# jamesdolezal/biscuit

Measured on NVIDIA B200. Metric: MC-dropout tiles/sec (Xception-UQ, T=30, 299^2), higher is better.
Workload: dtype bf16

## Files before the change

biscuit_b200/csrc/model.cu:

```cuda
#include <cuda.h>

#include <cmath>
#include <cstdlib>
#include <map>
#include <memory>

#include "common.cuh"
#include "gemm_sm100.cuh"
#include "layers.cuh"
#include "head_sm100.cuh"
#include "dwpipe_sm100.cuh"
#include "sepconv2d_sm100.cuh"
#include "sepmid_sm100.cuh"
#include "conv1_sm100.cuh"
#include "stain_sm100.cuh"

int bq_stain_launch(bq_ctx* ctx, const uint8_t* tiles_dev, int64_t n, int32_t px, const float* lut_dev, float* stats_dev,
                    const float target_means[3], const float target_stds[3], uint8_t* out_dev);

using bq::bf16;
using bq::GemmParams;

namespace {

// ... 131 lines not shown
    for (int c = 0; c < cin; ++c)
      for (int o = 0; o < cout; ++o)
        h[(size_t)o * ktot + t * cin + c] = f32_to_bf16_rne(k->data[((size_t)t * cin + c) * cout + o]);
  w.cin = cin; w.cout = cout; w.ktot = ktot;
  if ((rc = upload(ctx, w.w, h.data(), h.size() * 2))) return rc;
  return load_bn(ctx, ti, name + "_bn", cout, w);
}

int load_dense(bq_ctx* ctx, const TensorIndex& ti, const std::string& name, int cin, int cout, PwWeights& w) {
  const bq_named_tensor *k, *b;
  int rc;
  if ((rc = need(ctx, ti, name + "/kernel", {cin, cout}, &k)) || (rc = need(ctx, ti, name + "/bias", {cout}, &b))) return rc;
  std::vector<uint16_t> h((size_t)cout * cin);
  for (int c = 0; c < cin; ++c)
    for (int o = 0; o < cout; ++o) h[(size_t)o * cin + c] = f32_to_bf16_rne(k->data[(size_t)c * cout + o]);
  w.cin = cin; w.cout = cout; w.ktot = cin;
  if ((rc = upload(ctx, w.w, h.data(), h.size() * 2))) return rc;
  return upload(ctx, w.shift, b->data, cout * 4);
}

enum OpKind { OP_STATS, OP_CONV1, OP_GEMM, OP_DW, OP_POOLADD, OP_SUBSAMPLE, OP_GAP, OP_SEP2D, OP_SEPMID };

struct Op {
  OpKind kind;
  int stage = 0;
  std::string tag;
  const bf16* in = nullptr;
  const bf16* in2 = nullptr;
  bf16* out = nullptr;
  int H = 0, W = 0, C = 0, Ho = 0, Wo = 0, Cout = 0;
  int relu_in = 0, pad_top = 0, pad_left = 0;
  const float* dw = nullptr;
  bq::sep2d::Sep2dParams s2;
  bq::sepmid::SepMidParams sm;
  bool padded_out = false;
  int in_pitch = 0, out_pitch = 0;
  GemmParams gp;
  int rows_per_tile = 0;
  int blk_k = 64;
  CUtensorMap ta, tb, tc, tr;
  CUtensorMap tb2;
};

struct Arena {
  DevBuf buf[5];
  bf16* p(int i) { return (bf16*)buf[i].p; }
};

}

struct bq_model {
  bq_ctx* ctx = nullptr;
  bq_model_config cfg{};
  bool weights_loaded = false;
  bool use_simt = false;
  bool use_graph = true;
  cudaGraphExec_t backbone_graph = nullptr;
  int64_t graph_kernels = 0;
  bool sep_mid = true;
  DevBuf midbuf[4];
  int max_batch = 0;
  int px = 299;

  DevBuf conv1_w, conv1_scale, conv1_shift;
  DevBuf conv1_wtc, conv1_sumw;
  DevBuf conv1_affine, conv1_m0;
  PwWeights conv2;
  std::map<std::string, std::unique_ptr<SepWeights>> sep;
  std::map<std::string, std::unique_ptr<PwWeights>> res;
  std::vector<std::unique_ptr<PwWeights>> hidden;
  DevBuf w3, b3;

  DevBuf tiles_dev;
  DevBuf tiles_dev2;
  DevBuf tiles_f32[2];
  bool input_f32 = false;
  int norm_kind = 0;
  float norm_means[3] = {0, 0, 0}, norm_stds[3] = {1, 1, 1};
  DevBuf tiles_norm, norm_lut, norm_stats;
  const uint8_t* tiles_src = nullptr;
  cudaStream_t copy_stream = nullptr;
  cudaEvent_t copied[2] = {}, consumed[2] = {};
  DevBuf mean, inv_std;
  Arena arena;
  DevBuf feat, feat_bf16;
  DevBuf h_act[2];
  DevBuf a2;
  DevBuf a0;
  int sites = 6;
  int n_sites = 2, slot[3] = {-1, 0, 1};
  int mask_w = 0;
  DevBuf out_mean, out_std;
// ... 162 lines not shown
    if ((rc = make_tmap(ctx, &op.ta, A.p(0), (uint64_t)s1 * s1 * B, 32, 32, 128, 32))) return rc;
    if ((rc = make_tmap(ctx, &op.tb, m->conv2.w.p, 64, 288, 288, 64, 32))) return rc;
    if ((rc = make_tmap_nhwc(ctx, &op.tc, A.p(1), (uint64_t)B, (uint64_t)s2, (uint64_t)s2, 64, 1, 32, 32, false, true))) return rc;
    op.tr = op.ta; op.tb2 = op.tb;
    op.Ho = s2; op.Wo = s2; op.Cout = 64;
    m->plan.push_back(op);
  }
  X = 1;
  int H = s2, C = 64;

  int dw_rc = BQ_OK;
  int n_dw = 0;
  auto add_dw = [&](const bf16* in, bf16* out, int h, int c, int relu_in, const SepWeights& sw, int stage, int in_pitch = 0) {
    Op op; op.kind = OP_DW; op.stage = stage; op.in = in; op.out = out; op.H = h; op.W = h; op.C = c;
    op.relu_in = relu_in; op.dw = (const float*)sw.dw.p;
    const int CC = (c % 64 != 0) ? 56 : 64;
    int r = make_tmap_nhwc(ctx, &op.ta, in, (uint64_t)B, (uint64_t)h, (uint64_t)h, (uint64_t)c, bq::dwp::kHalo, bq::dwp::kHalo, CC,
                           false, false, (uint64_t)in_pitch);
    if (r && !dw_rc) dw_rc = r;
    op.tag = "dw" + std::to_string(n_dw++);
    op.Ho = h; op.Wo = h; op.Cout = c;
    m->plan.push_back(op);
  };
  auto add_gemm = [&](const bf16* a, int rows, const PwWeights& w, bf16* out, int relu, const bf16* resid, int stage,
                      const char* tag, int h, int cout) -> int {
    Op op; op.stage = stage;
    int r = make_gemm(m, op, a, rows, w, out, relu, resid);
    if (r) return r;
    if (tag) op.tag = tag;
    op.Ho = h; op.Wo = h; op.Cout = cout;
    m->plan.push_back(op);
    return BQ_OK;
  };
  auto add_sep = [&](const bf16* in, bf16* dw_tmp, int h, int cin, int relu_in, const SepWeights& sw, bf16* out, int relu_out,
                     const bf16* resid, int stage, const char* tag, int in_pitch = 0) -> int {
    if (!in_pitch && !m->use_simt && !resid && cin % 64 == 0 && cin <= 256 && (sw.pw.cout == 128 || sw.pw.cout == 256)) {
      Op op; op.kind = OP_SEP2D; op.stage = stage;
      if (tag) op.tag = tag;
      op.in = in; op.out = out; op.H = h; op.W = h; op.C = cin; op.Ho = h; op.Wo = h; op.Cout = sw.pw.cout;
      op.s2.n_img = B; op.s2.H = h; op.s2.W = h; op.s2.K = cin; op.s2.N = sw.pw.cout;
      op.s2.relu_in = relu_in; op.s2.relu_out = relu_out;
      op.s2.dw = (const float*)sw.dw.p; op.s2.scale = (const float*)sw.pw.scale.p; op.s2.shift = (const float*)sw.pw.shift.p;
      int r;
      if ((r = make_tmap_nhwc(ctx, &op.ta, in, (uint64_t)B, (uint64_t)h, (uint64_t)h, (uint64_t)cin, bq::sep2d::kHH, bq::sep2d::kHW, 64, false))) return r;
      if ((r = make_tmap(ctx, &op.tb, sw.pw.w.p, (uint64_t)sw.pw.cout, (uint64_t)cin, (uint64_t)cin, (uint32_t)sw.pw.cout, 64))) return r;
      if ((r = make_tmap_nhwc(ctx, &op.tc, out, (uint64_t)B, (uint64_t)h, (uint64_t)h, (uint64_t)sw.pw.cout, 2, bq::sep2d::kPW, 32, false, true))) return r;
      m->plan.push_back(op);
      return BQ_OK;
    }
    add_dw(in, dw_tmp, h, cin, relu_in, sw, stage, in_pitch);
    return add_gemm(dw_tmp, h * h, sw.pw, out, relu_out, resid, stage, tag, h, sw.pw.cout);
  };
  auto res_block = [&](int b, int cout1, int cout2, int relu_first, int stage, const bf16* padded_in = nullptr,
                       bf16* padded_out = nullptr) -> int {
    int t[4]; others(X, t);
    const int Ho = (H + 1) / 2;
    const bf16* xin = padded_in ? padded_in : A.p(X);
    const int in_pitch = padded_in ? bq::sepmid::kPitch : 0;
    const SepWeights& s1w = *m->sep.at("block" + std::to_string(b) + "_sepconv1");
    const SepWeights& s2w = *m->sep.at("block" + std::to_string(b) + "_sepconv2");
    const PwWeights& rw = *m->res.at("block" + std::to_string(b) + "_res");
    { Op op; op.kind = OP_SUBSAMPLE; op.stage = stage; op.in = xin; op.in_pitch = in_pitch; op.out = A.p(t[0]); op.H = H; op.W = H; op.Ho = Ho; op.Wo = Ho; op.C = C; m->plan.push_back(op); }
    int r;
    if ((r = add_gemm(A.p(t[0]), Ho * Ho, rw, A.p(t[1]), 0, nullptr, stage, nullptr, Ho, cout2))) return r;
    if ((r = add_sep(xin, A.p(t[0]), H, C, relu_first, s1w, A.p(t[2]), 1, nullptr, stage, nullptr, in_pitch))) return r;
    if ((r = add_sep(A.p(t[2]), A.p(t[0]), H, cout1, 0, s2w, A.p(t[3]), 0, nullptr, stage, nullptr))) return r;
    { Op op; op.kind = OP_POOLADD; op.stage = stage; op.in = A.p(t[3]); op.in2 = A.p(t[1]); op.out = padded_out ? padded_out : A.p(X);
      op.out_pitch = padded_out ? bq::sepmid::kPitch : 0; op.padded_out = padded_out != nullptr;
      op.H = H; op.W = H; op.Ho = Ho; op.Wo = Ho; op.C = cout2; op.Cout = cout2; op.pad_top = same_pad_before(H); op.pad_left = same_pad_before(H);
      op.tag = "block" + std::to_string(b); m->plan.push_back(op); }
    H = Ho; C = cout2;
    return BQ_OK;
  };
  if ((rc = res_block(2, 128, 128, 0, 2)) || (rc = res_block(3, 256, 256, 1, 2))) return rc;
  const bool mid = m->sep_mid && (H + 1) / 2 == bq::sepmid::kMap;
  auto P = [&](int i) { return (bf16*)m->midbuf[i].p; };
  if (mid) {
    using namespace bq::sepmid;
    const uint64_t rows = (uint64_t)B * kImgRows + kSlackRows;
    for (auto& b : m->midbuf) {
      if ((rc = bq_alloc(ctx, b, rows * kC * sizeof(bf16)))) return rc;
      BQ_CUDA(ctx, cudaMemset(b.p, 0, rows * kC * sizeof(bf16)));
    }
  }
  if ((rc = res_block(4, 728, 728, 1, 2, nullptr, mid ? P(0) : nullptr))) return rc;
  int mid_out = -1;
  if (mid) {
    using namespace bq::sepmid;
    const uint64_t rows = (uint64_t)B * kImgRows + kSlackRows;
    auto add_mid = [&](int src, int dst, int res, const SepWeights& sw, int relu_in, int relu_out, const char* tag) -> int {
      Op op; op.kind = OP_SEPMID; op.stage = 3; op.padded_out = true;
      if (tag) op.tag = tag;
      op.in = P(src); op.out = P(dst); op.in2 = res >= 0 ? P(res) : nullptr;
      op.H = kMap; op.W = kMap; op.C = kC; op.Ho = kMap; op.Wo = kMap; op.Cout = kC; op.relu_in = relu_in;
      op.sm.n_rows = B * kImgRows; op.sm.relu_out = relu_out;
      op.sm.dw = (const float*)sw.dw.p; op.sm.scale = (const float*)sw.pw.scale.p; op.sm.shift = (const float*)sw.pw.shift.p;
      op.sm.residual = op.in2;
      int r;
// ... 91 lines not shown
      KScope ks(m, g.conv_mode ? BQ_K_GEMM_CONV2 : BQ_K_GEMM_PW, 2.0 * rows_out * g.N * g.K,
                act * ((double)g.M * kin + rows_out * g.N * (g.residual ? 2 : 1) + (double)g.N * g.K));
      return launch_gemm(m, g, op.ta, op.tb, op.tc, op.tr, op.blk_k, g.conv_mode ? nullptr : &op.tb2);
    }
    case OP_DW: {
      KScope ks(m, BQ_K_DW, 2.0 * 9 * nb * op.H * op.W * op.C, 2 * act * nb * op.H * op.W * op.C);
      const int CC = (op.C % 64 != 0) ? 56 : 64;
      const int tiles = (op.H + bq::dwp::kTile - 1) / bq::dwp::kTile;
      const int64_t items = (int64_t)nb * tiles * tiles * (op.C / CC);
      const int grid = (int)std::min<int64_t>(items, ctx->num_sms);
#define BQ_DWP_LAUNCH(RELU, CCV)                                                                              \
  bq::dwp::depthwise3x3_pipe_kernel<RELU, CCV><<<grid, bq::dwp::kThreads, bq::dwp::kSmem, ctx->stream>>>(    \
      op.ta, op.dw, op.out, nb, op.H, op.W, op.C, tiles)
      if (CC == 56) { if (op.relu_in) BQ_DWP_LAUNCH(true, 56); else BQ_DWP_LAUNCH(false, 56); }
      else          { if (op.relu_in) BQ_DWP_LAUNCH(true, 64); else BQ_DWP_LAUNCH(false, 64); }
#undef BQ_DWP_LAUNCH
      break;
    }
    case OP_POOLADD: {
      KScope ks(m, BQ_K_POOLADD, 0, act * nb * op.C * ((double)op.H * op.W + 2.0 * op.Ho * op.Wo));
      bq::maxpool_add_kernel<<<grid1d((int64_t)nb * op.Ho * op.Wo * (op.C / 8)), 256, 0, ctx->stream>>>(
          op.in, op.in2, op.out + out_off, nb, op.H, op.W, op.Ho, op.Wo, op.C, op.pad_top, op.pad_left, op.out_pitch);
      break;
    }
    case OP_SUBSAMPLE: {
      KScope ks(m, BQ_K_SUBSAMPLE, 0, 2 * act * nb * op.Ho * op.Wo * op.C);
      bq::subsample2_kernel<<<grid1d((int64_t)nb * op.Ho * op.Wo * (op.C / 8)), 256, 0, ctx->stream>>>(
          op.in, op.out, nb, op.H, op.W, op.Ho, op.Wo, op.C, op.in_pitch);
      break;
    }
    case OP_SEP2D: {
      bq::sep2d::Sep2dParams s2 = op.s2;
      s2.n_img = nb;
      const int items = nb * ((op.H + bq::sep2d::kPH - 1) / bq::sep2d::kPH) * ((op.W + bq::sep2d::kPW - 1) / bq::sep2d::kPW);
      const int grid = items < ctx->num_sms ? items : ctx->num_sms;
      const double px_n = (double)nb * op.H * op.W;
      KScope ks(m, BQ_K_SEP_FUSED, 2.0 * px_n * s2.K * (s2.N + 9.0), act * px_n * (s2.K + s2.N));
      const int smem2d = bq::sep2d::smem_bytes(s2.N);
      if (s2.relu_in)
        bq::sep2d::sepconv2d_fused_kernel<true><<<grid, bq::sep2d::kThreads, smem2d, ctx->stream>>>(op.ta, op.tb, op.tc, s2);
      else
        bq::sep2d::sepconv2d_fused_kernel<false><<<grid, bq::sep2d::kThreads, smem2d, ctx->stream>>>(op.ta, op.tb, op.tc, s2);
      break;
    }
    case OP_SEPMID: {
      bq::sepmid::SepMidParams sm = op.sm;
      sm.n_rows = nb * bq::sepmid::kImgRows;
      const int items = (sm.n_rows + bq::sepmid::kItemPx - 1) / bq::sepmid::kItemPx;
      const int clusters = items < ctx->num_sms / 2 ? items : ctx->num_sms / 2;
      const double px_n = (double)nb * op.H * op.W;
      KScope ks(m, BQ_K_SEP_MID, 2.0 * px_n * op.C * (op.C + 9.0), act * px_n * op.C * (sm.residual ? 3.0 : 2.0));
      if (op.relu_in)
        bq::sepmid::sepconv_mid_kernel<true><<<2 * clusters, bq::sepmid::kThreads, bq::sepmid::kSmem, ctx->stream>>>(op.ta, op.tb, op.tc, op.tr, sm);
      else
        bq::sepmid::sepconv_mid_kernel<false><<<2 * clusters, bq::sepmid::kThreads, bq::sepmid::kSmem, ctx->stream>>>(op.ta, op.tb, op.tc, op.tr, sm);
      break;
    }
    case OP_GAP: {
      KScope ks(m, BQ_K_GAP, 0, act * nb * op.H * op.W * op.C + 6.0 * nb * op.C);
      bq::gap_kernel<<<grid1d((int64_t)nb * op.C), 256, 0, ctx->stream>>>(op.in, (float*)m->feat.p,
                                                                           (bf16*)m->feat_bf16.p, nb, op.H * op.W, op.C);
      break;
    }
  }
  BQ_LAUNCH_CHECK(ctx);
  return BQ_OK;
}

int stage_tiles(bq_model* m, const uint8_t* tiles, int nb) {
  bq_ctx* ctx = m->ctx;
  const size_t bytes = (size_t)nb * m->px * m->px * 3;
  BQ_CUDA(ctx, cudaMemcpyAsync(m->tiles_dev.p, tiles, bytes, cudaMemcpyDefault, ctx->stream));
  m->tiles_src = (const uint8_t*)m->tiles_dev.p;
  return BQ_OK;
}
// ... 153 lines not shown
    out[i] = __bfloat162float(in[i]);
}

}

extern "C" {

int bq_model_create(bq_ctx* ctx, const bq_model_config* cfg, bq_model** out) {
  if (!ctx) return BQ_ERR_ARG;
  if (!cfg || !out) return bq_fail(ctx, BQ_ERR_ARG, "bq_model_create: null argument");
  if (cfg->tile_px != 299) return bq_fail(ctx, BQ_ERR_ARG, "tile_px must be 299 (hp.py:5), got %d", cfg->tile_px);
  if (cfg->hidden_layers != 2) return bq_fail(ctx, BQ_ERR_ARG, "hidden_layers must be 2 (hp.py:21), got %d", cfg->hidden_layers);
  if (cfg->hidden_width <= 0 || cfg->hidden_width % 64) return bq_fail(ctx, BQ_ERR_ARG, "hidden_width must be a positive multiple of 64");
  if (cfg->n_classes < 2 || cfg->n_classes > bq::kMaxClasses) return bq_fail(ctx, BQ_ERR_ARG, "n_classes must be in [2,8]");
  if (!(cfg->dropout >= 0.f && cfg->dropout < 1.f)) return bq_fail(ctx, BQ_ERR_ARG, "dropout must be in [0,1)");
  if (cfg->max_batch < 1 || cfg->max_batch > 512) return bq_fail(ctx, BQ_ERR_ARG, "max_batch must be in [1,512]");
  BQ_CUDA(ctx, cudaSetDevice(ctx->device));
  bq_model* m = new bq_model();
  m->ctx = ctx;
  m->cfg = *cfg;
  m->max_batch = cfg->max_batch;
  m->px = cfg->tile_px;
  m->sites = cfg->dropout_sites ? cfg->dropout_sites : 6;
  if (m->sites & ~7) { delete m; return bq_fail(ctx, BQ_ERR_ARG, "dropout_sites must be a bitmask of sites 0..2"); }
  m->n_sites = 0;
  for (int i = 0; i < 3; ++i) m->slot[i] = (m->sites >> i) & 1 ? m->n_sites++ : -1;
  m->mask_w = (m->sites & 1) ? kFeatures : cfg->hidden_width;
  const char* g = getenv("BQ_GEMM");
  m->use_simt = g && strcmp(g, "simt") == 0;
  const char* gr = getenv("BQ_GRAPH");
  m->use_graph = !(gr && strcmp(gr, "off") == 0);
  const char* smid = getenv("BQ_SEPMID");
  m->sep_mid = !(smid && strcmp(smid, "off") == 0) && !m->use_simt;
  using namespace bq::sm100;
  cudaFuncSetAttribute(gemm_tcgen05_2cta_kernel<k2Stages>, cudaFuncAttributeMaxDynamicSharedMemorySize, SmemPlan2<k2Stages>::kTotal);
  cudaFuncSetAttribute(gemm_tcgen05_2cta_kernel<k2Stages + 1>, cudaFuncAttributeMaxDynamicSharedMemorySize, SmemPlan2<k2Stages + 1>::kTotalNoRes);
  cudaFuncSetAttribute(conv3x3_is_kernel, cudaFuncAttributeMaxDynamicSharedMemorySize, kC2Smem);
  cudaFuncSetAttribute(bq::conv1tc::conv1_tc_kernel, cudaFuncAttributeMaxDynamicSharedMemorySize, bq::conv1tc::kSmem);
  cudaFuncSetAttribute(bq::head::mc_head_fused_kernel, cudaFuncAttributeMaxDynamicSharedMemorySize, bq::head::HeadSmem::kTotal);
  cudaFuncSetAttribute(bq::sep2d::sepconv2d_fused_kernel<true>, cudaFuncAttributeMaxDynamicSharedMemorySize, bq::sep2d::smem_bytes(256));
  cudaFuncSetAttribute(bq::sep2d::sepconv2d_fused_kernel<false>, cudaFuncAttributeMaxDynamicSharedMemorySize, bq::sep2d::smem_bytes(256));
  cudaFuncSetAttribute(bq::sepmid::sepconv_mid_kernel<true>, cudaFuncAttributeMaxDynamicSharedMemorySize, bq::sepmid::kSmem);
  cudaFuncSetAttribute(bq::sepmid::sepconv_mid_kernel<false>, cudaFuncAttributeMaxDynamicSharedMemorySize, bq::sepmid::kSmem);
  cudaFuncSetAttribute(bq::dwp::depthwise3x3_pipe_kernel<true, 56>, cudaFuncAttributeMaxDynamicSharedMemorySize, bq::dwp::kSmem);
  cudaFuncSetAttribute(bq::dwp::depthwise3x3_pipe_kernel<false, 56>, cudaFuncAttributeMaxDynamicSharedMemorySize, bq::dwp::kSmem);
  cudaFuncSetAttribute(bq::dwp::depthwise3x3_pipe_kernel<true, 64>, cudaFuncAttributeMaxDynamicSharedMemorySize, bq::dwp::kSmem);
  cudaFuncSetAttribute(bq::dwp::depthwise3x3_pipe_kernel<false, 64>, cudaFuncAttributeMaxDynamicSharedMemorySize, bq::dwp::kSmem);
  for (auto& e : m->ev) cudaEventCreate(&e);
  cudaStreamCreateWithFlags(&m->copy_stream, cudaStreamNonBlocking);
  for (int i = 0; i < 2; ++i) {
    cudaEventCreateWithFlags(&m->copied[i], cudaEventDisableTiming);
    cudaEventCreateWithFlags(&m->consumed[i], cudaEventDisableTiming);
  }
  cudaError_t e = cudaGetLastError();
  if (e != cudaSuccess) { delete m; return bq_fail(ctx, BQ_ERR_CUDA, "cudaFuncSetAttribute: %s", cudaGetErrorString(e)); }
  *out = m;
  return BQ_OK;
}

void bq_model_destroy(bq_model* m) {
  if (!m) return;
  cudaSetDevice(m->ctx->device);
  cudaStreamSynchronize(m->ctx->stream);
  if (m->backbone_graph) cudaGraphExecDestroy(m->backbone_graph);
  for (auto& e : m->ev) if (e) cudaEventDestroy(e);
  for (auto& e : m->kev) cudaEventDestroy(e);
  if (m->copy_stream) { cudaStreamSynchronize(m->copy_stream); cudaStreamDestroy(m->copy_stream); }
  for (int i = 0; i < 2; ++i) { if (m->copied[i]) cudaEventDestroy(m->copied[i]); if (m->consumed[i]) cudaEventDestroy(m->consumed[i]); }
  delete m;
}

int bq_model_load_weights(bq_model* m, const bq_named_tensor* tensors, int32_t n_tensors) {
  if (!m) return BQ_ERR_ARG;
  bq_ctx* ctx = m->ctx;
// ... 309 lines not shown
```

biscuit_b200/csrc/sepconv2d_sm100.cuh:

```cuda
#pragma once

#include "gemm_sm100.cuh"

namespace bq {
namespace sep2d {

using namespace sm100;

constexpr int kPH = 8, kPW = 16;
constexpr int kHH = kPH + 2, kHW = kPW + 2;
constexpr int kPatchBytes = 23 * 1024;
constexpr int kABytes = 128 * 128;
constexpr int kOutTile = 32 * 64;
constexpr int kOutBufs = 2;
constexpr int kOutBytes = 8 * kOutBufs * kOutTile;
constexpr int kMaxPStages = 5, kAStages = 2, kBStages = 2;
constexpr int kOffPatch = 0;
__host__ __device__ inline int patch_stages(int N) { (void)N; return 4; }
__host__ __device__ inline int off_a(int N) { return patch_stages(N) * kPatchBytes; }
__host__ __device__ inline int off_b(int N) { return off_a(N) + kAStages * kABytes; }
__host__ __device__ inline int off_out(int N) { return off_b(N) + kBStages * N * 128; }
__host__ __device__ inline int off_scale(int N) { return off_out(N) + kOutBytes; }
__host__ __device__ inline int off_bar(int N) { return off_scale(N) + 2 * 256 * 4; }
__host__ __device__ inline int smem_bytes(int N) { return off_bar(N) + 512 + 1024; }
constexpr int kThreads = 576;
constexpr int kProducerWarps = 8;

struct Sep2dParams {
  int n_img, H, W;
  int K, N;
  int relu_in, relu_out;
  const float* dw;
  const float* scale;
  const float* shift;
};

template <bool RELU_IN>
__global__ void __launch_bounds__(kThreads, 1)
sepconv2d_fused_kernel(const __grid_constant__ CUtensorMap tmap_x ,
                       const __grid_constant__ CUtensorMap tmap_w ,
                       const __grid_constant__ CUtensorMap tmap_out ,
                       const Sep2dParams p) {
  extern __shared__ uint8_t smem_raw[];
  const uint32_t smem_base = (smem_u32(smem_raw) + 1023u) & ~1023u;
  uint8_t* smem_gen = smem_raw + (smem_base - smem_u32(smem_raw));
  const int kPStages = patch_stages(p.N);
  const int kOffA = off_a(p.N), kOffB = off_b(p.N), kOffOut = off_out(p.N), kOffScale = off_scale(p.N), kOffBar = off_bar(p.N);
  const int kBBytes = p.N * 128;
  const uint32_t bar0 = smem_base + kOffBar;
  auto patch_full = [&](int s) { return bar0 + 8u * s; };
  auto patch_empty = [&](int s) { return bar0 + 8u * (5 + s); };
  auto a_full = [&](int s) { return bar0 + 8u * (10 + s); };
  auto a_empty = [&](int s) { return bar0 + 8u * (12 + s); };
  auto b_full = [&](int s) { return bar0 + 8u * (14 + s); };
  auto b_empty = [&](int s) { return bar0 + 8u * (16 + s); };
  auto acc_full = [&](int s) { return bar0 + 8u * (18 + s); };
  auto acc_empty = [&](int s) { return bar0 + 8u * (20 + s); };
  const uint32_t tmem_slot = bar0 + 8u * 22;
  volatile uint32_t* tmem_slot_ptr = (volatile uint32_t*)(smem_gen + kOffBar + 8 * 22);
  float* s_scale = (float*)(smem_gen + kOffScale);
  float* s_shift = s_scale + 256;

  const int warp = uniform_warp_idx(), lane = threadIdx.x & 31;
  const int px_tiles = (p.W + kPW - 1) / kPW, py_tiles = (p.H + kPH - 1) / kPH;
  const int per_img = px_tiles * py_tiles;
  const int n_items = p.n_img * per_img;
  const int num_kb = p.K / 64;
  const uint32_t b_bytes = (uint32_t)p.N * 128u;
  const bool b_resident = num_kb <= kBStages;

  if (threadIdx.x == 0) {
    tma_prefetch_desc(&tmap_x);
    tma_prefetch_desc(&tmap_w);
    tma_prefetch_desc(&tmap_out);
    for (int s = 0; s < kPStages; ++s) { mbar_init(patch_full(s), 1); mbar_init(patch_empty(s), kProducerWarps / 2); }
    for (int s = 0; s < 2; ++s) {
      mbar_init(a_full(s), kProducerWarps / 2); mbar_init(a_empty(s), 1);
      mbar_init(b_full(s), 1); mbar_init(b_empty(s), 1);
      mbar_init(acc_full(s), 1); mbar_init(acc_empty(s), 8);
    }
    asm volatile("fence.mbarrier_init.release.cluster;" ::: "memory");
  }
  for (int i = threadIdx.x; i < p.N; i += blockDim.x) { s_scale[i] = __ldg(p.scale + i); s_shift[i] = __ldg(p.shift + i); }
  if (warp == 1) tmem_alloc(tmem_slot, 512);
  tc_fence_before();
  __syncthreads();
  tc_fence_after();
  const uint32_t tmem_base = __shfl_sync(0xffffffffu, *tmem_slot_ptr, 0);

  if (warp == 0) {
    if (lane == 0) {
      int ps = 0; uint32_t pph = 0;
      int bs = 0; uint32_t bph = 0;
      if (b_resident) {
        for (int st = 0; st < kBStages; ++st) {
          mbar_expect_tx(b_full(st), b_bytes);
          tma_load_2d(smem_base + kOffB + st * kBBytes, &tmap_w, b_full(st), (st % num_kb) * 64, 0);
        }
      }
      for (int it = blockIdx.x; it < n_items; it += gridDim.x) {
        const int img = it / per_img, t = it - img * per_img;
        const int y0 = (t / px_tiles) * kPH, x0 = (t % px_tiles) * kPW;
        for (int kb = 0; kb < num_kb; ++kb) {
          mbar_wait(patch_empty(ps), pph ^ 1u);
          mbar_expect_tx(patch_full(ps), (uint32_t)(kHH * kHW * 128));
          asm volatile(
              "cp.async.bulk.tensor.4d.shared::cluster.global.mbarrier::complete_tx::bytes [%0], [%1, {%3, %4, %5, %6}], [%2];"
              ::"r"(smem_base + kOffPatch + ps * kPatchBytes), "l"((uint64_t)&tmap_x), "r"(patch_full(ps)), "r"(kb * 64),
                "r"(x0 - 1), "r"(y0 - 1), "r"(img)
              : "memory");
          if (++ps == kPStages) { ps = 0; pph ^= 1u; }
          if (b_resident) continue;
          mbar_wait(b_empty(bs), bph ^ 1u);
          mbar_expect_tx(b_full(bs), b_bytes);
          tma_load_2d(smem_base + kOffB + bs * kBBytes, &tmap_w, b_full(bs), kb * 64, 0);
          if (++bs == kBStages) { bs = 0; bph ^= 1u; }
        }
      }
    }
  } else if (warp == 1) {
    {
      const uint32_t idesc = make_idesc(128, 128);
      const int n_ct = p.N >> 7;
      int as = 0; uint32_t aph = 0;
      int cs = 0; uint32_t cph = 0;
      int gk = 0;
      for (int it = blockIdx.x; it < n_items; it += gridDim.x) {
        mbar_wait(acc_empty(cs), cph ^ 1u);
#pragma unroll 1
        for (int kb = 0; kb < num_kb; ++kb) {
          mbar_wait(a_full(as), aph);
          if (!b_resident || gk < kBStages) mbar_wait(b_full(as), aph);
          ++gk;
          tc_fence_after();
          const uint64_t dpx = make_smem_desc<128>(smem_base + kOffA + as * kABytes);
          const uint64_t dw0 = make_smem_desc<128>(smem_base + kOffB + as * kBBytes);
          if (elect_one()) {
            for (int ct = 0; ct < n_ct; ++ct) {
              const uint64_t dw = dw0 + (uint64_t)(ct * ((128 * 128) >> 4));
              const uint32_t d = tmem_base + (uint32_t)(cs * 256 + ct * 128);
              umma_bf16(d, dw, dpx, idesc, kb ? 1u : 0u);
              umma_bf16(d, dw + 2u, dpx + 2u, idesc, 1u);
              umma_bf16(d, dw + 4u, dpx + 4u, idesc, 1u);
              umma_bf16(d, dw + 6u, dpx + 6u, idesc, 1u);
            }
            umma_commit(a_empty(as));
            if (!b_resident) umma_commit(b_empty(as));
            if (kb == num_kb - 1) umma_commit(acc_full(cs));
          }
          __syncwarp();
          if (++as == 2) { as = 0; aph ^= 1u; }
        }
        if (++cs == 2) { cs = 0; cph ^= 1u; }
      }
    }
  } else if (warp < 10) {
    const int quad = warp & 3;
    const int hh = (warp - 2) >> 2;
    const int w8 = warp - 2;
    const int n_ct = p.N >> 7;
    const uint32_t my_out = smem_base + kOffOut + (uint32_t)(w8 * kOutBufs * kOutTile);
    const int mrow = lane & 7, mmat = lane >> 3;
    int cs = 0; uint32_t cph = 0;
    uint32_t g = 0;
    for (int it = blockIdx.x; it < n_items; it += gridDim.x) {
      const int img = it / per_img, t = it - img * per_img;
      const int y0 = (t / px_tiles) * kPH, x0 = (t % px_tiles) * kPW;
      mbar_wait(acc_full(cs), cph);
      tc_fence_after();
      for (int ct = 0; ct < n_ct; ++ct) {
        float s4[4], h4[4];
#pragma unroll
        for (int k = 0; k < 4; ++k) {
          const int c = ct * 128 + quad * 32 + (lane >> 2) + 8 * k;
          s4[k] = s_scale[c];
          h4[k] = s_shift[c];
        }
        const uint32_t t_lo = tmem_base + ((uint32_t)(quad * 32) << 16) + (uint32_t)(cs * 256 + ct * 128 + hh * 64);
        const uint32_t t_hi = t_lo + (16u << 16);
#pragma unroll
        for (int s2 = 0; s2 < 2; ++s2, ++g) {
          uint32_t lo[16], hi[16];
          tmem_ld_16x256b_x4(t_lo + (uint32_t)(s2 * 32), lo);
          tmem_ld_16x256b_x4(t_hi + (uint32_t)(s2 * 32), hi);
          tmem_ld_wait();
          if (ct == n_ct - 1 && s2 == 1) {
            tc_fence_before();
            __syncwarp();
            if (lane == 0) mbar_arrive(acc_empty(cs));
          }
          uint32_t pkv[16];
#pragma unroll
          for (int b = 0; b < 4; ++b) {
            float f[8];
#pragma unroll
            for (int k = 0; k < 2; ++k) {
              f[2 * k] = __fadd_rn(__fmul_rn(__uint_as_float(lo[4 * b + 2 * k]), s4[k]), h4[k]);
              f[2 * k + 1] = __fadd_rn(__fmul_rn(__uint_as_float(lo[4 * b + 2 * k + 1]), s4[k]), h4[k]);
              f[4 + 2 * k] = __fadd_rn(__fmul_rn(__uint_as_float(hi[4 * b + 2 * k]), s4[2 + k]), h4[2 + k]);
              f[4 + 2 * k + 1] = __fadd_rn(__fmul_rn(__uint_as_float(hi[4 * b + 2 * k + 1]), s4[2 + k]), h4[2 + k]);
// ... 12 lines not shown
          fence_async_smem();
          __syncwarp();
          if (elect_one()) {
            asm volatile("cp.async.bulk.tensor.4d.global.shared::cta.bulk_group [%0, {%2, %3, %4, %5}], [%1];"
                         ::"l"((uint64_t)&tmap_out), "r"(stg), "r"(ct * 128 + quad * 32), "r"(x0), "r"(y0 + hh * 4 + s2 * 2), "r"(img)
                         : "memory");
            tma_store_commit();
          }
          __syncwarp();
        }
      }
      if (++cs == 2) { cs = 0; cph ^= 1u; }
    }
    if (elect_one()) tma_store_wait_all();
    __syncwarp();
  } else {
    const int ptid = threadIdx.x - 320;
    const int grp = ptid >> 7, tg = ptid & 127;
    const int c4 = tg & 15, pair = tg >> 4;
    auto load4 = [&](const uint8_t* rowp, float2 (&d)[4][2]) {
#pragma unroll
      for (int k = 0; k < 4; ++k) {
        uint2 raw = *(const uint2*)(rowp + (size_t)k * 128);
        if (RELU_IN) {
          const __nv_bfloat162 z2 = __floats2bfloat162_rn(0.f, 0.f);
          __nv_bfloat162* hb = (__nv_bfloat162*)&raw;
          hb[0] = __hmax2(hb[0], z2);
          hb[1] = __hmax2(hb[1], z2);
        }
        d[k][0] = make_float2(__uint_as_float(raw.x << 16), __uint_as_float(raw.x & 0xFFFF0000u));
        d[k][1] = make_float2(__uint_as_float(raw.y << 16), __uint_as_float(raw.y & 0xFFFF0000u));
      }
    };
    const int total_kb = ((n_items - (int)blockIdx.x + (int)gridDim.x - 1) / (int)gridDim.x) * num_kb;
    for (int q = grp; q < total_kb; q += 2) {
      const int kb = q % num_kb;
      const int ps = q % kPStages;
      const uint32_t pph = (uint32_t)(q / kPStages) & 1u, aph = (uint32_t)(q >> 1) & 1u;
      const int c = kb * 64 + c4 * 4;
      float2 w[9][2];
#pragma unroll
      for (int t = 0; t < 9; ++t) {
        const float4 wv = __ldg((const float4*)(p.dw + (size_t)t * p.K + c));
        w[t][0] = make_float2(wv.x, wv.y);
        w[t][1] = make_float2(wv.z, wv.w);
      }
      if (q > 0) mbar_wait(patch_full((q - 1) % kPStages), (uint32_t)((q - 1) / kPStages) & 1u);
      mbar_wait(patch_full(ps), pph);
      mbar_wait(a_empty(grp), aph ^ 1u);
      const uint8_t* col = smem_gen + kOffPatch + ps * kPatchBytes + (size_t)(2 * pair) * 128 + c4 * 8;
      uint8_t* a_dst = smem_gen + kOffA + grp * kABytes;
      float2 ra[4][2], rb[4][2], rc[4][2];
      load4(col, ra);
      load4(col + (size_t)kHW * 128, rb);
      auto step = [&](const float2 (&r0)[4][2], const float2 (&r1)[4][2], float2 (&r2)[4][2], int py) {
        load4(col + (size_t)(py + 2) * kHW * 128, r2);
        float2 a[2][2];
        a[0][0] = a[0][1] = a[1][0] = a[1][1] = make_float2(0.f, 0.f);
#pragma unroll
        for (int kx = 0; kx < 3; ++kx)
#pragma unroll
          for (int h = 0; h < 2; ++h) {
            a[0][h] = __ffma2_rn(r0[kx][h], w[kx][h], a[0][h]);
            a[1][h] = __ffma2_rn(r0[kx + 1][h], w[kx][h], a[1][h]);
          }
#pragma unroll
        for (int kx = 0; kx < 3; ++kx)
// ... 41 lines not shown
```

Baseline: 26050.

## Fuse 3x3/2 max-pool and residual add into second sepconv2d epilogue

In entry-flow residual blocks, the second separable conv now runs a pooled variant of the fused sep2d kernel. Its epilogue applies BN, does a stride-2 3x3 max-pool across tiles using carried rows and warp shuffles, and adds the residual loaded by TMA. The result is stored directly as the pooled block output. This removes the separate pool-add kernel and the full-resolution intermediate write and read. In exchange, work is scheduled as vertical strips walked in row order so the pool window can carry between tiles, which changes load balance and adds epilogue complexity.

```diff
diff --git a/biscuit_b200/csrc/model.cu b/biscuit_b200/csrc/model.cu
--- a/biscuit_b200/csrc/model.cu
+++ b/biscuit_b200/csrc/model.cu
@@ -187,6 +187,7 @@
   int relu_in = 0, pad_top = 0, pad_left = 0;
   const float* dw = nullptr;
   bq::sep2d::Sep2dParams s2;
+  bool pool = false;
   bq::sepmid::SepMidParams sm;
   bool padded_out = false;
   int in_pitch = 0, out_pitch = 0;
@@ -213,6 +214,7 @@
   cudaGraphExec_t backbone_graph = nullptr;
   int64_t graph_kernels = 0;
   bool sep_mid = true;
+  bool pool_fuse = true;
   DevBuf midbuf[4];
   int max_batch = 0;
   int px = 299;
@@ -441,19 +443,27 @@
     m->plan.push_back(op);
     return BQ_OK;
   };
+  auto sep2d_fits = [&](int cin, int cout) { return !m->use_simt && cin % 64 == 0 && cin <= 256 && (cout == 128 || cout == 256); };
+  auto sep2d_op = [&](Op& op, const bf16* in, int h, int cin, int relu_in, const SepWeights& sw, int relu_out, int stage) -> int {
+    op.kind = OP_SEP2D; op.stage = stage;
+    op.in = in; op.H = h; op.W = h; op.C = cin; op.Ho = h; op.Wo = h; op.Cout = sw.pw.cout;
+    op.s2.n_img = B; op.s2.H = h; op.s2.W = h; op.s2.K = cin; op.s2.N = sw.pw.cout;
+    op.s2.relu_in = relu_in; op.s2.relu_out = relu_out; op.s2.pool_pad = 0;
+    op.s2.dw = (const float*)sw.dw.p; op.s2.scale = (const float*)sw.pw.scale.p; op.s2.shift = (const float*)sw.pw.shift.p;
+    int r;
+    if ((r = make_tmap_nhwc(ctx, &op.ta, in, (uint64_t)B, (uint64_t)h, (uint64_t)h, (uint64_t)cin, bq::sep2d::kHH, bq::sep2d::kHW, 64, false))) return r;
+    return make_tmap(ctx, &op.tb, sw.pw.w.p, (uint64_t)sw.pw.cout, (uint64_t)cin, (uint64_t)cin, (uint32_t)sw.pw.cout, 64);
+  };
   auto add_sep = [&](const bf16* in, bf16* dw_tmp, int h, int cin, int relu_in, const SepWeights& sw, bf16* out, int relu_out,
                      const bf16* resid, int stage, const char* tag, int in_pitch = 0) -> int {
-    if (!in_pitch && !m->use_simt && !resid && cin % 64 == 0 && cin <= 256 && (sw.pw.cout == 128 || sw.pw.cout == 256)) {
-      Op op; op.kind = OP_SEP2D; op.stage = stage;
+    if (!in_pitch && !resid && sep2d_fits(cin, sw.pw.cout)) {
+      Op op;
+      int r;
+      if ((r = sep2d_op(op, in, h, cin, relu_in, sw, relu_out, stage))) return r;
       if (tag) op.tag = tag;
-      op.in = in; op.out = out; op.H = h; op.W = h; op.C = cin; op.Ho = h; op.Wo = h; op.Cout = sw.pw.cout;
-      op.s2.n_img = B; op.s2.H = h; op.s2.W = h; op.s2.K = cin; op.s2.N = sw.pw.cout;
-      op.s2.relu_in = relu_in; op.s2.relu_out = relu_out;
-      op.s2.dw = (const float*)sw.dw.p; op.s2.scale = (const float*)sw.pw.scale.p; op.s2.shift = (const float*)sw.pw.shift.p;
-      int r;
-      if ((r = make_tmap_nhwc(ctx, &op.ta, in, (uint64_t)B, (uint64_t)h, (uint64_t)h, (uint64_t)cin, bq::sep2d::kHH, bq::sep2d::kHW, 64, false))) return r;
-      if ((r = make_tmap(ctx, &op.tb, sw.pw.w.p, (uint64_t)sw.pw.cout, (uint64_t)cin, (uint64_t)cin, (uint32_t)sw.pw.cout, 64))) return r;
+      op.out = out;
       if ((r = make_tmap_nhwc(ctx, &op.tc, out, (uint64_t)B, (uint64_t)h, (uint64_t)h, (uint64_t)sw.pw.cout, 2, bq::sep2d::kPW, 32, false, true))) return r;
+      op.tr = op.tc;
       m->plan.push_back(op);
       return BQ_OK;
     }
@@ -473,6 +483,19 @@
     int r;
     if ((r = add_gemm(A.p(t[0]), Ho * Ho, rw, A.p(t[1]), 0, nullptr, stage, nullptr, Ho, cout2))) return r;
     if ((r = add_sep(xin, A.p(t[0]), H, C, relu_first, s1w, A.p(t[2]), 1, nullptr, stage, nullptr, in_pitch))) return r;
+    if (m->pool_fuse && !padded_out && sep2d_fits(cout1, cout2)) {
+      Op op;
+      if ((r = sep2d_op(op, A.p(t[2]), H, cout1, 0, s2w, 0, stage))) return r;
+      op.out = A.p(X); op.in2 = A.p(t[1]); op.Ho = Ho; op.Wo = Ho; op.pool = true;
+      op.s2.pool_pad = same_pad_before(H);
+      op.tag = "block" + std::to_string(b);
+      using namespace bq::sep2d;
+      if ((r = make_tmap_nhwc(ctx, &op.tc, op.out, (uint64_t)B, (uint64_t)Ho, (uint64_t)Ho, (uint64_t)cout2, kPoolRows, kPoolCols, kPoolCh))) return r;
+      if ((r = make_tmap_nhwc(ctx, &op.tr, op.in2, (uint64_t)B, (uint64_t)Ho, (uint64_t)Ho, (uint64_t)cout2, kPoolRows, kPoolCols, kPoolCh))) return r;
+      m->plan.push_back(op);
+      H = Ho; C = cout2;
+      return BQ_OK;
+    }
     if ((r = add_sep(A.p(t[2]), A.p(t[0]), H, cout1, 0, s2w, A.p(t[3]), 0, nullptr, stage, nullptr))) return r;
     { Op op; op.kind = OP_POOLADD; op.stage = stage; op.in = A.p(t[3]); op.in2 = A.p(t[1]); op.out = padded_out ? padded_out : A.p(X);
       op.out_pitch = padded_out ? bq::sepmid::kPitch : 0; op.padded_out = padded_out != nullptr;
@@ -630,15 +653,19 @@
     case OP_SEP2D: {
       bq::sep2d::Sep2dParams s2 = op.s2;
       s2.n_img = nb;
-      const int items = nb * ((op.H + bq::sep2d::kPH - 1) / bq::sep2d::kPH) * ((op.W + bq::sep2d::kPW - 1) / bq::sep2d::kPW);
-      const int grid = items < ctx->num_sms ? items : ctx->num_sms;
+      const int units = op.pool ? nb * bq::sep2d::pool_strips(op.W)
+                                : nb * ((op.H + bq::sep2d::kPH - 1) / bq::sep2d::kPH) * ((op.W + bq::sep2d::kPW - 1) / bq::sep2d::kPW);
+      const int grid = units < ctx->num_sms ? units : ctx->num_sms;
       const double px_n = (double)nb * op.H * op.W;
-      KScope ks(m, BQ_K_SEP_FUSED, 2.0 * px_n * s2.K * (s2.N + 9.0), act * px_n * (s2.K + s2.N));
+      const double out_bytes = op.pool ? 2.0 * act * nb * op.Ho * op.Wo * s2.N : act * px_n * s2.N;
+      KScope ks(m, BQ_K_SEP_FUSED, 2.0 * px_n * s2.K * (s2.N + 9.0), act * px_n * s2.K + out_bytes);
       const int smem2d = bq::sep2d::smem_bytes(s2.N);
-      if (s2.relu_in)
-        bq::sep2d::sepconv2d_fused_kernel<true><<<grid, bq::sep2d::kThreads, smem2d, ctx->stream>>>(op.ta, op.tb, op.tc, s2);
+      if (op.pool)
+        bq::sep2d::sepconv2d_fused_kernel<false, true><<<grid, bq::sep2d::kThreads, smem2d, ctx->stream>>>(op.ta, op.tb, op.tc, op.tr, s2);
+      else if (s2.relu_in)
+        bq::sep2d::sepconv2d_fused_kernel<true, false><<<grid, bq::sep2d::kThreads, smem2d, ctx->stream>>>(op.ta, op.tb, op.tc, op.tr, s2);
       else
-        bq::sep2d::sepconv2d_fused_kernel<false><<<grid, bq::sep2d::kThreads, smem2d, ctx->stream>>>(op.ta, op.tb, op.tc, s2);
+        bq::sep2d::sepconv2d_fused_kernel<false, false><<<grid, bq::sep2d::kThreads, smem2d, ctx->stream>>>(op.ta, op.tb, op.tc, op.tr, s2);
       break;
     }
     case OP_SEPMID: {
@@ -858,14 +885,17 @@
   m->use_graph = !(gr && strcmp(gr, "off") == 0);
   const char* smid = getenv("BQ_SEPMID");
   m->sep_mid = !(smid && strcmp(smid, "off") == 0) && !m->use_simt;
+  const char* pf = getenv("BQ_POOLFUSE");
+  m->pool_fuse = !(pf && strcmp(pf, "off") == 0);
   using namespace bq::sm100;
   cudaFuncSetAttribute(gemm_tcgen05_2cta_kernel<k2Stages>, cudaFuncAttributeMaxDynamicSharedMemorySize, SmemPlan2<k2Stages>::kTotal);
   cudaFuncSetAttribute(gemm_tcgen05_2cta_kernel<k2Stages + 1>, cudaFuncAttributeMaxDynamicSharedMemorySize, SmemPlan2<k2Stages + 1>::kTotalNoRes);
   cudaFuncSetAttribute(conv3x3_is_kernel, cudaFuncAttributeMaxDynamicSharedMemorySize, kC2Smem);
   cudaFuncSetAttribute(bq::conv1tc::conv1_tc_kernel, cudaFuncAttributeMaxDynamicSharedMemorySize, bq::conv1tc::kSmem);
   cudaFuncSetAttribute(bq::head::mc_head_fused_kernel, cudaFuncAttributeMaxDynamicSharedMemorySize, bq::head::HeadSmem::kTotal);
-  cudaFuncSetAttribute(bq::sep2d::sepconv2d_fused_kernel<true>, cudaFuncAttributeMaxDynamicSharedMemorySize, bq::sep2d::smem_bytes(256));
-  cudaFuncSetAttribute(bq::sep2d::sepconv2d_fused_kernel<false>, cudaFuncAttributeMaxDynamicSharedMemorySize, bq::sep2d::smem_bytes(256));
+  cudaFuncSetAttribute(bq::sep2d::sepconv2d_fused_kernel<true, false>, cudaFuncAttributeMaxDynamicSharedMemorySize, bq::sep2d::smem_bytes(256));
+  cudaFuncSetAttribute(bq::sep2d::sepconv2d_fused_kernel<false, false>, cudaFuncAttributeMaxDynamicSharedMemorySize, bq::sep2d::smem_bytes(256));
+  cudaFuncSetAttribute(bq::sep2d::sepconv2d_fused_kernel<false, true>, cudaFuncAttributeMaxDynamicSharedMemorySize, bq::sep2d::smem_bytes(256));
   cudaFuncSetAttribute(bq::sepmid::sepconv_mid_kernel<true>, cudaFuncAttributeMaxDynamicSharedMemorySize, bq::sepmid::kSmem);
   cudaFuncSetAttribute(bq::sepmid::sepconv_mid_kernel<false>, cudaFuncAttributeMaxDynamicSharedMemorySize, bq::sepmid::kSmem);
   cudaFuncSetAttribute(bq::dwp::depthwise3x3_pipe_kernel<true, 56>, cudaFuncAttributeMaxDynamicSharedMemorySize, bq::dwp::kSmem);
diff --git a/biscuit_b200/csrc/sepconv2d_sm100.cuh b/biscuit_b200/csrc/sepconv2d_sm100.cuh
--- a/biscuit_b200/csrc/sepconv2d_sm100.cuh
+++ b/biscuit_b200/csrc/sepconv2d_sm100.cuh
@@ -25,22 +25,75 @@
 __host__ __device__ inline int smem_bytes(int N) { return off_bar(N) + 512 + 1024; }
 constexpr int kThreads = 576;
 constexpr int kProducerWarps = 8;
+constexpr int kPoolRows = kPH / 2, kPoolCols = 7, kPoolCh = 16;
+constexpr int kPoolTile = kPoolRows * kPoolCols * kPoolCh * 2;
+constexpr int kPoolGroups = 2;
+constexpr int kPoolWarpBytes = kOutBytes / 8;
+static_assert(kPoolGroups * 2 * kPoolTile <= kPoolWarpBytes && kPoolTile % 128 == 0, "pooled tiles must fit the staging area");
 
 struct Sep2dParams {
   int n_img, H, W;
   int K, N;
   int relu_in, relu_out;
+  int pool_pad;
   const float* dw;
   const float* scale;
   const float* shift;
 };
 
-template <bool RELU_IN>
+__host__ __device__ inline int pool_strips(int W) { return ((W + 1) / 2 + kPoolCols - 1) / kPoolCols; }
+
+template <bool POOL>
+struct Items {
+  int px_tiles, py_tiles, n;
+  __device__ explicit Items(const Sep2dParams& p) {
+    py_tiles = (p.H + kPH - 1) / kPH;
+    px_tiles = POOL ? pool_strips(p.W) : (p.W + kPW - 1) / kPW;
+    const int units = p.n_img * px_tiles * (POOL ? 1 : py_tiles);
+    const int mine = units > (int)blockIdx.x ? (units - (int)blockIdx.x + (int)gridDim.x - 1) / (int)gridDim.x : 0;
+    n = POOL ? mine * py_tiles : mine;
+  }
+  __device__ void coords(const Sep2dParams& p, int li, int& img, int& y0, int& x0) const {
+    if (POOL) {
+      const int s = (int)blockIdx.x + (li / py_tiles) * (int)gridDim.x;
+      img = s / px_tiles;
+      y0 = (li % py_tiles) * kPH;
+      x0 = (s % px_tiles) * (2 * kPoolCols) - p.pool_pad;
+    } else {
+      const int it = (int)blockIdx.x + li * (int)gridDim.x;
+      const int per_img = px_tiles * py_tiles;
+      img = it / per_img;
+      const int t = it - img * per_img;
+      y0 = (t / px_tiles) * kPH;
+      x0 = (t % px_tiles) * kPW;
+    }
+  }
+};
+
+__device__ __forceinline__ uint32_t hmax_bf16x2(uint32_t a, uint32_t b) {
+  const __nv_bfloat162 r = __hmax2(*reinterpret_cast<const __nv_bfloat162*>(&a), *reinterpret_cast<const __nv_bfloat162*>(&b));
+  return *reinterpret_cast<const uint32_t*>(&r);
+}
+__device__ __forceinline__ void tma_load_4d(uint32_t smem_dst, const CUtensorMap* tmap, uint32_t bar, int c0, int c1, int c2, int c3) {
+  asm volatile(
+      "cp.async.bulk.tensor.4d.shared::cluster.global.mbarrier::complete_tx::bytes [%0], [%1, {%3, %4, %5, %6}], [%2];"
+      ::"r"(smem_dst), "l"((uint64_t)tmap), "r"(bar), "r"(c0), "r"(c1), "r"(c2), "r"(c3)
+      : "memory");
+}
+__device__ __forceinline__ void tma_store_4d(const CUtensorMap* tmap, uint32_t smem_src, int c0, int c1, int c2, int c3) {
+  asm volatile("cp.async.bulk.tensor.4d.global.shared::cta.bulk_group [%0, {%2, %3, %4, %5}], [%1];"
+               ::"l"((uint64_t)tmap), "r"(smem_src), "r"(c0), "r"(c1), "r"(c2), "r"(c3)
+               : "memory");
+}
+
+template <bool RELU_IN, bool POOL>
 __global__ void __launch_bounds__(kThreads, 1)
 sepconv2d_fused_kernel(const __grid_constant__ CUtensorMap tmap_x ,
                        const __grid_constant__ CUtensorMap tmap_w ,
                        const __grid_constant__ CUtensorMap tmap_out ,
+                       const __grid_constant__ CUtensorMap tmap_res ,
                        const Sep2dParams p) {
+  static_assert(!(POOL && RELU_IN), "the pooled layers take already-ReLU'd input");
   extern __shared__ uint8_t smem_raw[];
   const uint32_t smem_base = (smem_u32(smem_raw) + 1023u) & ~1023u;
   uint8_t* smem_gen = smem_raw + (smem_base - smem_u32(smem_raw));
@@ -56,15 +109,14 @@
   auto b_empty = [&](int s) { return bar0 + 8u * (16 + s); };
   auto acc_full = [&](int s) { return bar0 + 8u * (18 + s); };
   auto acc_empty = [&](int s) { return bar0 + 8u * (20 + s); };
+  auto res_full = [&](int w8, int b, int ct) { return bar0 + 8u * (24 + 2 * (kPoolGroups * w8 + b) + ct); };
   const uint32_t tmem_slot = bar0 + 8u * 22;
   volatile uint32_t* tmem_slot_ptr = (volatile uint32_t*)(smem_gen + kOffBar + 8 * 22);
   float* s_scale = (float*)(smem_gen + kOffScale);
   float* s_shift = s_scale + 256;
 
   const int warp = uniform_warp_idx(), lane = threadIdx.x & 31;
-  const int px_tiles = (p.W + kPW - 1) / kPW, py_tiles = (p.H + kPH - 1) / kPH;
-  const int per_img = px_tiles * py_tiles;
-  const int n_items = p.n_img * per_img;
+  const Items<POOL> items(p);
   const int num_kb = p.K / 64;
   const uint32_t b_bytes = (uint32_t)p.N * 128u;
   const bool b_resident = num_kb <= kBStages;
@@ -73,12 +125,16 @@
     tma_prefetch_desc(&tmap_x);
     tma_prefetch_desc(&tmap_w);
     tma_prefetch_desc(&tmap_out);
+    if (POOL) tma_prefetch_desc(&tmap_res);
     for (int s = 0; s < kPStages; ++s) { mbar_init(patch_full(s), 1); mbar_init(patch_empty(s), kProducerWarps / 2); }
     for (int s = 0; s < 2; ++s) {
       mbar_init(a_full(s), kProducerWarps / 2); mbar_init(a_empty(s), 1);
       mbar_init(b_full(s), 1); mbar_init(b_empty(s), 1);
       mbar_init(acc_full(s), 1); mbar_init(acc_empty(s), 8);
     }
+    if (POOL)
+      for (int w8 = 0; w8 < 8; ++w8)
+        for (int b = 0; b < kPoolGroups; ++b) { mbar_init(res_full(w8, b, 0), 1); mbar_init(res_full(w8, b, 1), 1); }
     asm volatile("fence.mbarrier_init.release.cluster;" ::: "memory");
   }
   for (int i = threadIdx.x; i < p.N; i += blockDim.x) { s_scale[i] = __ldg(p.scale + i); s_shift[i] = __ldg(p.shift + i); }
@@ -98,9 +154,9 @@
           tma_load_2d(smem_base + kOffB + st * kBBytes, &tmap_w, b_full(st), (st % num_kb) * 64, 0);
         }
       }
-      for (int it = blockIdx.x; it < n_items; it += gridDim.x) {
-        const int img = it / per_img, t = it - img * per_img;
-        const int y0 = (t / px_tiles) * kPH, x0 = (t % px_tiles) * kPW;
+      for (int li = 0; li < items.n; ++li) {
+        int img, y0, x0;
+        items.coords(p, li, img, y0, x0);
         for (int kb = 0; kb < num_kb; ++kb) {
           mbar_wait(patch_empty(ps), pph ^ 1u);
           mbar_expect_tx(patch_full(ps), (uint32_t)(kHH * kHW * 128));
@@ -125,7 +181,7 @@
       int as = 0; uint32_t aph = 0;
       int cs = 0; uint32_t cph = 0;
       int gk = 0;
-      for (int it = blockIdx.x; it < n_items; it += gridDim.x) {
+      for (int li = 0; li < items.n; ++li) {
         mbar_wait(acc_empty(cs), cph ^ 1u);
 #pragma unroll 1
         for (int kb = 0; kb < num_kb; ++kb) {
@@ -154,6 +210,125 @@
         if (++cs == 2) { cs = 0; cph ^= 1u; }
       }
     }
+  } else if (POOL && warp < 10) {
+    const int quad = warp & 3, hh = (warp - 2) >> 2, w8 = warp - 2;
+    const int n_ct = p.N >> 7;
+    const int g8 = lane >> 2, j = lane & 3;
+    const int ch0 = quad * 32 + hh * 16;
+    constexpr uint32_t kNegInf = 0xFF80FF80u;
+    const uint32_t stg = smem_base + kOffOut + (uint32_t)(w8 * kPoolWarpBytes);
+    uint16_t* const stg_gen = (uint16_t*)(smem_gen + kOffOut + w8 * kPoolWarpBytes);
+    auto tile = [&](int li, int ct) { return (uint32_t)(((li % kPoolGroups) * 2 + ct) * kPoolTile); };
+    auto res_load = [&](int li, int ct) {
+      int img, y0, x0;
+      items.coords(p, li, img, y0, x0);
+      if (elect_one()) {
+        tma_store_wait_read0();
+        mbar_expect_tx(res_full(w8, li % kPoolGroups, ct), (uint32_t)kPoolTile);
+        tma_load_4d(stg + tile(li, ct), &tmap_res, res_full(w8, li % kPoolGroups, ct), ct * 128 + ch0, (x0 + p.pool_pad) >> 1, y0 >> 1, img);
+      }
+      __syncwarp();
+    };
+    auto store = [&](int li, int ct) {
+      int img, y0, x0;
+      items.coords(p, li, img, y0, x0);
+      fence_async_smem();
+      __syncwarp();
+      if (elect_one()) {
+        tma_store_4d(&tmap_out, stg + tile(li, ct), ct * 128 + ch0, (x0 + p.pool_pad) >> 1, y0 >> 1, img);
+        tma_store_commit();
+      }
+      __syncwarp();
+    };
+    auto finish_row = [&](int li, int ct, int k, uint32_t oa, uint32_t ob) {
+      uint16_t* row = stg_gen + (tile(li, ct) >> 1) + k * kPoolCols * kPoolCh + g8;
+      auto fin = [&](uint16_t* px, uint32_t o) {
+        const float r0 = __uint_as_float((uint32_t)px[0] << 16), r1 = __uint_as_float((uint32_t)px[8] << 16);
+        const uint32_t q = pack_bf16x2(__fadd_rn(__uint_as_float(o << 16), r0), __fadd_rn(__uint_as_float(o & 0xFFFF0000u), r1), false);
+        px[0] = (uint16_t)q;
+        px[8] = (uint16_t)(q >> 16);
+      };
+      fin(row + j * kPoolCh, oa);
+      if (j < 3) fin(row + (4 + j) * kPoolCh, ob);
+    };
+    uint32_t carry_a[2] = {kNegInf, kNegInf}, carry_b[2] = {kNegInf, kNegInf};
+    int cs = 0; uint32_t cph = 0;
+    if (items.n > 0)
+      for (int ct = 0; ct < n_ct; ++ct) res_load(0, ct);
+    for (int li = 0; li < items.n; ++li) {
+      int img, y0, x0;
+      items.coords(p, li, img, y0, x0);
+      const bool first = y0 == 0, last = y0 + kPH >= p.H;
+      const bool col_edge = x0 < 0 || x0 + kPW > p.W;
+      bool col_ok[4];
+#pragma unroll
+      for (int i = 0; i < 4; ++i) {
+        const int x = x0 + 8 * (i >> 1) + 2 * j + (i & 1);
+        col_ok[i] = x >= 0 && x < p.W;
+      }
+      mbar_wait(acc_full(cs), cph);
+      tc_fence_after();
+#pragma unroll
+      for (int ct = 0; ct < 2; ++ct) {
+        if (ct == n_ct) break;
+        mbar_wait(res_full(w8, li % kPoolGroups, ct), (uint32_t)(li / kPoolGroups) & 1u);
+        const int c = ct * 128 + ch0 + g8;
+        const float s0 = s_scale[c], s1 = s_scale[c + 8], h0 = s_shift[c], h1 = s_shift[c + 8];
+        auto hpool = [&](const uint32_t* v, int y, uint32_t& ha, uint32_t& hb) {
+          if (y >= p.H) { ha = hb = kNegInf; return; }
+          float f[8];
+#pragma unroll
+          for (int i = 0; i < 8; ++i) f[i] = __fadd_rn(__fmul_rn(__uint_as_float(v[i]), (i & 2) ? s1 : s0), (i & 2) ? h1 : h0);
+          uint32_t e[2] = {pack_bf16x2(f[0], f[2], false), pack_bf16x2(f[4], f[6], false)};
+          uint32_t o[2] = {pack_bf16x2(f[1], f[3], false), pack_bf16x2(f[5], f[7], false)};
+          if (col_edge) {
+            e[0] = col_ok[0] ? e[0] : kNegInf; o[0] = col_ok[1] ? o[0] : kNegInf;
+            e[1] = col_ok[2] ? e[1] : kNegInf; o[1] = col_ok[3] ? o[1] : kNegInf;
+          }
+          const uint32_t na = __shfl_sync(0xffffffffu, j == 0 ? e[1] : e[0], j < 3 ? lane + 1 : lane - 3);
+          const uint32_t nb = __shfl_sync(0xffffffffu, e[1], (lane + 1) & 31);
+          ha = hmax_bf16x2(hmax_bf16x2(e[0], o[0]), na);
+          hb = hmax_bf16x2(hmax_bf16x2(e[1], o[1]), nb);
+        };
+        const uint32_t t0 = tmem_base + ((uint32_t)ch0 << 16) + (uint32_t)(cs * 256 + ct * 128);
+        uint32_t ca = first ? kNegInf : carry_a[ct], cb = first ? kNegInf : carry_b[ct];
+#pragma unroll
+        for (int k = 0; k < kPoolRows; ++k) {
+          uint32_t v[16];
+          tmem_ld_16x256b_x4(t0 + (uint32_t)(k * 32), v);
+          tmem_ld_wait();
+          if (ct == n_ct - 1 && k == kPoolRows - 1) {
+            tc_fence_before();
+            __syncwarp();
+            if (lane == 0) mbar_arrive(acc_empty(cs));
+          }
+          {
+            uint32_t a0, b0, a1, b1;
+            hpool(v, y0 + 2 * k, a0, b0);
+            hpool(v + 8, y0 + 2 * k + 1, a1, b1);
+            if (p.pool_pad) {
+              finish_row(li, ct, k, hmax_bf16x2(hmax_bf16x2(ca, a0), a1), hmax_bf16x2(hmax_bf16x2(cb, b0), b1));
+              ca = a1; cb = b1;
+            } else {
+              if (k > 0) {
+                finish_row(li, ct, k - 1, hmax_bf16x2(ca, a0), hmax_bf16x2(cb, b0));
+              } else if (!first) {
+                finish_row(li - 1, ct, kPoolRows - 1, hmax_bf16x2(ca, a0), hmax_bf16x2(cb, b0));
+                store(li - 1, ct);
+              }
+              ca = hmax_bf16x2(a0, a1); cb = hmax_bf16x2(b0, b1);
+            }
+            if (k == 0 && li + 1 < items.n) res_load(li + 1, ct);
+          }
+        }
+        if (!p.pool_pad && last) finish_row(li, ct, kPoolRows - 1, ca, cb);
+        if (p.pool_pad || last) store(li, ct);
+        carry_a[ct] = ca; carry_b[ct] = cb;
+      }
+      if (++cs == 2) { cs = 0; cph ^= 1u; }
+    }
+    if (elect_one()) tma_store_wait_all();
+    __syncwarp();
   } else if (warp < 10) {
     const int quad = warp & 3;
     const int hh = (warp - 2) >> 2;
@@ -163,9 +338,9 @@
     const int mrow = lane & 7, mmat = lane >> 3;
     int cs = 0; uint32_t cph = 0;
     uint32_t g = 0;
-    for (int it = blockIdx.x; it < n_items; it += gridDim.x) {
-      const int img = it / per_img, t = it - img * per_img;
-      const int y0 = (t / px_tiles) * kPH, x0 = (t % px_tiles) * kPW;
+    for (int li = 0; li < items.n; ++li) {
+      int img, y0, x0;
+      items.coords(p, li, img, y0, x0);
       mbar_wait(acc_full(cs), cph);
       tc_fence_after();
       for (int ct = 0; ct < n_ct; ++ct) {
@@ -244,7 +419,7 @@
         d[k][1] = make_float2(__uint_as_float(raw.y << 16), __uint_as_float(raw.y & 0xFFFF0000u));
       }
     };
-    const int total_kb = ((n_items - (int)blockIdx.x + (int)gridDim.x - 1) / (int)gridDim.x) * num_kb;
+    const int total_kb = items.n * num_kb;
     for (int q = grp; q < total_kb; q += 2) {
       const int kb = q % num_kb;
       const int ps = q % kPStages;
```

After: 26560 (median of 6 runs). 1.02x the previous value.
